# Plachtaa/FAcodec

Hardware: AMD Instinct MI355X
Metric: 24kHz audio sec encoded+decoded per wall-sec (higher is better)
Workload: dtype f32; 1 GPU; configs[1]: batch=32/GPU x 2 s @ 24 kHz, forward encoder->FVQ(6 codebooks)->decoder, FAcodec configs/config.yml model (137.7 M params), weights formula-generated, weight-norm re-materialised every step; clips_per_gpu=32, samples_per_clip=48000, parallelism=dp1 (independent clips, no collective)

## Files before the change

### facodec_amd/_lib.py

```python
import ctypes as C
import os

_HERE = os.path.dirname(os.path.abspath(__file__))
LIB_PATH = os.environ.get("FAC_LIB_PATH", os.path.join(_HERE, "libfacodec_hip.so"))

PAD_ZERO, PAD_REFLECT = 0, 1
ACT_NONE, ACT_TANH, ACT_MISH, ACT_LOG_MEL = 0, 1, 2, 3
ACT_GATE, ACT_WN_RES_SKIP = 4, 5

_p = C.c_void_p
_i = C.c_int
_i64 = C.c_int64
_f = C.c_float


class ConvDesc(C.Structure):
    _fields_ = [
        ("x", _p), ("w", _p), ("bias", _p), ("alpha_in", _p), ("alpha_out", _p), ("res", _p), ("y", _p), ("y2", _p), ("alpha_y2", _p), ("w_k1", _p), ("bias_k1", _p),
        ("x_bs", _i64), ("x_cs", _i64), ("y_bs", _i64), ("y_cs", _i64),
        ("B", C.c_int32), ("C_in", C.c_int32), ("T_in", C.c_int32), ("C_out", C.c_int32),
        ("C_out_pad", C.c_int32), ("T_out", C.c_int32),
        ("K", C.c_int32), ("stride", C.c_int32), ("dilation", C.c_int32), ("pad_left", C.c_int32),
        ("pad_mode", C.c_int32), ("n_phase", C.c_int32), ("y_tstride", C.c_int32), ("phase_shift", C.c_int32),
        ("act", C.c_int32),
        ("w_batched", C.c_int32), ("w_bs", _i64), ("ws", _p), ("ws_bytes", _i64), ("w_split", _p),
        ("K1", C.c_int32), ("dilation2", C.c_int32), ("row_phases", C.c_int32),
        ("x_p8", _p), ("x_p8_plane_bytes", _i64), ("y2_p8", _p), ("y2_p8_plane_bytes", _i64),
        ("pw_split", C.c_int32), ("split_rows", C.c_int32),
        ("gate_cond", _p), ("gate_cond_bs", _i64),
    ]


class VqDesc(C.Structure):
    _fields_ = [
        ("residual", _p), ("z_in", _p), ("zq_acc", _p), ("zq_out", _p), ("w_in", _p), ("b_in", _p),
        ("codebook", _p), ("w_out", _p), ("w_out_scale", _p), ("b_out", _p), ("mask", _p), ("codes", _p), ("z_e", _p),
        ("loss_part", _p), ("codes_bs", _i64),
        ("B", C.c_int32), ("D", C.c_int32), ("T", C.c_int32), ("Kc", C.c_int32),
    ]



VQ_DECODE_MAX_Q = 16


class VqDecodeDesc(C.Structure):
    _fields_ = [
        ("codes", _p * 3), ("codes_bs", _i64 * 3), ("codes_qs", _i64 * 3), ("n_q", C.c_int32 * 3),
        ("codebook", _p * VQ_DECODE_MAX_Q), ("w_out", _p * VQ_DECODE_MAX_Q), ("w_out_scale", _p * VQ_DECODE_MAX_Q),
        ("b_out", _p * VQ_DECODE_MAX_Q), ("style", _p), ("outs", _p), ("z", _p * 3),
        ("B", C.c_int32), ("D", C.c_int32), ("T", C.c_int32), ("Kc", C.c_int32),
# ... 258 lines not shown
```

### facodec_amd/build.py

```python
import os
import subprocess
import sys
from concurrent.futures import ThreadPoolExecutor

HERE = os.path.dirname(os.path.abspath(__file__))
CSRC = os.path.join(HERE, "csrc")
TAG = os.environ.get("FAC_BUILD_TAG", "")
LIB = os.path.join(HERE, "libfacodec_hip%s.so" % ("_" + TAG if TAG else ""))
OBJDIR = "build" + ("_" + TAG if TAG else "")
SOURCES = ["conv1d_api.hip", "conv1d_tile_128x128.hip", "conv1d_tile_96x128.hip", "conv1d_tile_64x128.hip",
           "conv1d_tile_32x256.hip", "conv1d_tile_128x32.hip", "conv1d_tile_128x256.hip", "conv1d_fused_ru.hip", "conv1d_narrow.hip", "conv1d_pw.hip", "conv1d_pw_split.hip", "conv1d_skinny.hip", "conv1d_bsplit.hip", "conv1d_bsplit96.hip", "conv1d_gemm_split.hip", "conv1d_bsplit2.hip", "conv1d_bwd.hip", "conv1d_wgrad_split.hip", "conv1d_wgrad_k1.hip", "train_misc.hip", "optim.hip", "train_quant.hip", "train_pred.hip", "train_disc.hip", "train_redecoder.hip", "pack.hip", "prep_batch.hip", "lstm.hip", "lstm_persist.hip", "vq.hip", "vq_decode.hip", "bitpack.hip", "misc.hip", "attention_stream.hip", "ragged.hip", "resample.hip", "loudness.hip", "metrics.hip", "stream_pool.hip", "jdc.hip", "rccl_arena.hip"]
FLAGS = ["--offload-arch=gfx950", "-O3", "-std=c++17", "-fPIC", "-ffp-contract=off",
         "-Wno-unused-result"] + os.environ.get("FAC_EXTRA_FLAGS", "").split()


def _hipcc():
    for cand in (os.environ.get("HIPCC"), "/opt/rocm/bin/hipcc", "hipcc"):
        if cand and (os.path.isabs(cand) and os.path.exists(cand) or not os.path.isabs(cand)):
            return cand
    return "hipcc"


def _stale(target, deps):
    if not os.path.exists(target):
        return True
    tt = os.path.getmtime(target)
    return any(os.path.getmtime(d) > tt for d in deps)


def build_lib(force=False, verbose=True):
    hipcc = _hipcc()
    headers = sorted(os.path.join(CSRC, f) for f in os.listdir(CSRC) if f.endswith(".h")) + [os.path.join(HERE, "..", "include", "facodec_hip.h")]
    objs, jobs = [], []
    os.makedirs(os.path.join(CSRC, OBJDIR), exist_ok=True)
# ... 23 lines not shown
```

### facodec_amd/convplan.py

```python
from collections import namedtuple

__all__ = ["ConvPlan", "ConvTrPlan", "plan_conv", "plan_convtr", "plan_gemm", "tile_rows", "gemm_split_ok", "gemm_split_strided_ok", "split2_ok",
           "pw_taps_ok", "pw_split_tail_ok", "convtr_split_ok", "convtr_rows_ok", "flat_strided_ok", "flat_convtr_ok", "W_FP32", "W_TAPS",
           "W_GEMM", "W_GEMM_STRIDED", "W_SPLIT2", "W_FP32_PW_TAPS", "PER_CLIP", "FLAT_STRIDED", "FLAT_STRIDE1", "TR_POLYPHASE", "TR_ROWS",
           "TR_ROWS_SPLIT", "TR_ROWS_PW_TAPS", "TR_FLAT"]

W_FP32, W_TAPS, W_GEMM, W_GEMM_STRIDED, W_SPLIT2, W_FP32_PW_TAPS = "fp32", "split_taps", "split_gemm", "split_gemm_strided", "split2", "fp32_pw_taps"
PER_CLIP, FLAT_STRIDED, FLAT_STRIDE1 = "per_clip", "flat_strided", "flat_stride1"
ConvPlan = namedtuple("ConvPlan", "layout form p8")
TR_POLYPHASE, TR_ROWS, TR_ROWS_SPLIT, TR_ROWS_PW_TAPS, TR_FLAT = "polyphase", "rows", "rows_split", "rows_pw_taps", "flat_rows_split"
ConvTrPlan = namedtuple("ConvTrPlan", "layout p8")


def _sw():
    from . import ops
    return ops


def gemm_split_ok(c_out, c_in, k, n_cols, t_out=None):
    sw = _sw()
    if not (sw.BF16_SPLIT and k in (1, 2)):
        return False
    if c_in < sw.GEMM_SPLIT_MIN_CIN or c_out < 64 or n_cols < 1024:
        return False
    return k == 1 or (t_out is not None and t_out >= 256)
# ... 27 lines not shown

def convtr_rows_ok(t_in, stride, causal=True):
    sw = _sw()
    return sw.CONVTR_ROWS and causal and 2 <= stride <= 16 and t_in >= sw.CONVTR_ROWS_MIN_T


def convtr_split_ok(c_in, c_out, stride, batch, t_in, causal=True, alpha_in=None):
    return (_sw().BF16_SPLIT and causal and alpha_in is None and 2 <= stride <= 16 and c_in >= 64
            and t_in >= 256 and batch * t_in >= 1024 and c_out * stride >= 64)


def flat_strided_ok(c_out, c_in, k, s, batch, n_out):
    return (_sw().FLAT_TRAIN and k == 2 * s and s > 1 and n_out < 256 and not gemm_split_strided_ok(c_out, c_in, k, s, batch, n_out)
            and gemm_split_strided_ok(c_out, c_in, k, s, 1, batch * (n_out + 1) - 1))


def flat_convtr_ok(c_in, c_out, s, batch, t_cols):
    return (_sw().FLAT_TRAIN and t_cols < 256 and not convtr_split_ok(c_in, c_out, s, batch, t_cols)
            and convtr_split_ok(c_in, c_out, s, 1, batch * t_cols))


def tile_rows(c_out, c_in, k, grad=False):
    sw = _sw()
    return 96 if (sw.BF16_SPLIT and not grad and k == 7 and c_out in sw.BS_ROWS96 and c_in % 8 == 0) else 64


def plan_conv(c_out, c_in, k, stride, dilation, batch, t_in, t_out, *, k1=0, alpha_in=False, plain=True, res=False,
              causal_reflect=False, grad=True, c_out_mult16=True, split_k=(1, 3, 5, 7), floor_k=(3, 5), tail="pw_split",
              pw_taps=True, split2=False, flat_infer=False, flat_stride1=False, flat_train=None):
    sw = _sw()
    cols = batch * t_out
    p8 = 2.0 * c_out * k / (4.0 * stride)
    if split2 and split2_ok(c_out, k, k1, stride, cols):
        return ConvPlan(W_SPLIT2, PER_CLIP, None)
    if stride > 1:
        strided = not alpha_in and dilation == 1 and not k1
        flat_t = (flat_train is not None and strided and plain and t_in % stride == 0
                  and (flat_train == "zero" or (causal_reflect and t_in > stride))
                  and flat_strided_ok(c_out, c_in, k, stride, batch, t_out))
        if flat_t and flat_train == "reflect":
            return ConvPlan(W_GEMM_STRIDED, FLAT_STRIDED, p8)
        if pw_taps and stride == 2 and strided and plain and pw_taps_ok(c_in, c_out, k, 2, False, batch, t_out):
            return ConvPlan(W_FP32_PW_TAPS, PER_CLIP, None)
        if strided and gemm_split_strided_ok(c_out, c_in, k, stride, batch, t_out):
            return ConvPlan(W_GEMM_STRIDED, PER_CLIP, p8)
        if flat_t:
            return ConvPlan(W_GEMM_STRIDED, FLAT_STRIDED, p8)
# ... 35 lines not shown
```

### facodec_amd/csrc/conv1d_api.hip

```cpp
#include "conv1d_mfma.h"
#include <stdlib.h>

namespace fac {

enum ConvKernel : int {
  CK_128x32 = 0,
  CK_32x256 = 1,
  CK_64x128 = 2,
  CK_96x128 = 3,
  CK_128x128 = 4,
  CK_128x256 = 5,
  CK_96x256 = 6,
  CK_FUSED_RU = 7,
  CK_128x160 = 8,
  CK_NARROW = 9,
  CK_SKINNY = 10,
  CK_BSPLIT = 11,
  CK_CIN1 = 12,
  CK_THIN = 13,
  CK_PW = 14,
  CK_GSPLIT = 15,
  CK_BSPLIT2 = 16,
  CK_PWS = 17,
  CK_PWT = 18,
// ... 41 lines not shown
  FAC_REQUIRE(!d->y2_p8 || d->alpha_y2, "conv1d: y2_p8 needs alpha_y2");
  if (d->w_k1) {
    FAC_REQUIRE(d->C_in == d->C_out && d->C_out_pad == d->C_out && d->n_phase == 1 && d->stride == 1 &&
                    d->alpha_out && d->act == FAC_ACT_NONE && !d->w_batched,
                "conv1d: fused ResidualUnit needs C_in == C_out (multiple of 32), stride 1, a Snake alpha_out");
  }
  a.x_bs = d->x_bs; a.x_cs = d->x_cs; a.y_bs = d->y_bs; a.y_cs = d->y_cs; a.w_bs = d->w_bs;
  a.B = d->B; a.C_in = d->C_in; a.T_in = d->T_in; a.C_out = d->C_out; a.C_out_pad = d->C_out_pad;
  a.T_out = d->T_out; a.K = d->K; a.stride = d->stride; a.dil = d->dilation;
  a.pad_left = d->pad_left; a.pad_mode = d->pad_mode; a.n_phase = d->n_phase;
  a.y_tstride = d->y_tstride; a.act = d->act; a.w_batched = d->w_batched;
  a.phase_shift = d->phase_shift;
  a.rp = d->row_phases > 1 ? d->row_phases : 1;
  FAC_REQUIRE(!d->gate_cond || (d->act == FAC_ACT_GATE && d->gate_cond_bs >= 0),
              "conv1d: gate_cond is the conditioning row of the FAC_ACT_GATE epilogue (act=%d gate_cond_bs=%lld)", d->act,
              (long long)d->gate_cond_bs);
  a.gate_cond = d->gate_cond; a.gate_cond_bs = d->gate_cond_bs;
  if (a.rp > 1) {
    FAC_REQUIRE(d->n_phase == 1 && d->y_tstride == 1 && d->phase_shift == 0 && d->stride == 1 && a.rp <= 128 && !d->w_k1 &&
                    !d->w_batched && d->C_out_pad == fac_convtr_rows(d->C_out, a.rp) && !(d->K1 > 0 && d->K1 < d->K),
                "conv1d: row_phases needs a plain stride-1 launch on weights from fac_pack_convtr_w_rows");
  }
  a.K1 = d->K1 > 0 ? d->K1 : d->K; a.dil2 = d->dilation2;
  FAC_REQUIRE(a.K1 <= d->K && d->K % a.K1 == 0 && (a.K1 == d->K || d->dilation2 > 0), "conv1d: bad two-level taps (K=%d K1=%d)", d->K, d->K1);
  FAC_REQUIRE(!conv_two_level(a) || (!d->w_k1 && d->n_phase == 1 && d->pad_mode == FAC_PAD_ZERO && !d->w_batched),
              "conv1d: two-level taps need a plain, zero-padded conv");
  conv_set_virtual(a);
  FAC_REQUIRE(d->phase_shift >= 0 && d->phase_shift < d->n_phase + (d->n_phase == 1), "conv1d: bad phase_shift");
  {
    long long last = (long long)(d->T_out - 1) * d->stride + (long long)conv_max_tap_offset(a) - d->pad_left;
    int pad_right = last >= d->T_in ? (int)(last - d->T_in + 1) : 0;
    int max_pad = d->pad_left > pad_right ? d->pad_left : pad_right;
    a.T_ext = d->T_in > max_pad ? d->T_in : max_pad + 1;
  }
  if (d->x_p8 || d->y2_p8) {
    const bool gs = d->w_split && (d->K <= 2 || (d->stride > 1 && d->K <= 2 * d->stride)) && conv_gsplit_ok(a) &&
                    !conv_skinny_ok(a, d->ws, d->ws_bytes) && d->C_in % 8 == 0 && d->x_p8_plane_bytes < (1ll << 32);
    const bool ok = !d->y2_p8 && (gs || (d->w_split && !conv_two_level(a) && (d->split_rows == 96 ? conv_bsplit96_p8_ok(a) : conv_bsplit_p8_ok(a)) &&
                                       !conv_cin1_ok(a)));
    FAC_REQUIRE(ok, "conv1d: P8 operands given but the launch does not run on a kernel that takes them (K=%d stride=%d C_in=%d columns=%lld)",
                d->K, d->stride, d->C_in, (long long)d->B * d->T_out);
  }
  if (d->act == FAC_ACT_GATE || d->act == FAC_ACT_WN_RES_SKIP) {
    FAC_REQUIRE(d->w && !d->w_k1 && !d->x_p8 && !conv_two_level(a) && conv_skinny_ok(a, d->ws, d->ws_bytes),
                "conv1d: FAC_ACT_GATE / FAC_ACT_WN_RES_SKIP exist only for few-column launches (B * T_out <= 640) with a workspace");
    k = CK_SKINNY;
// ... 3 lines not shown
  a.gflat = 0;
  a.grt = 0;
  if (d->w_split && (a.KV == 9 || a.KV == 3) && d->C_out <= 32 && conv_bsplit2_ok(a)) {
    a.w = reinterpret_cast<const float*>(d->w_split);
    k = CK_BSPLIT2;
    return FAC_OK;
  }
  FAC_REQUIRE(!conv_two_level(a) || d->w, "conv1d: two-level taps outside the split kernel's shapes need fp32 weights");
  const bool pw_on = pw_enabled();
  if (pw_on && d->pw_split && d->w && conv_pwt_ok(a)) { k = CK_PWT; return FAC_OK; }
  if (d->w_split && (d->K <= 2 || (d->stride > 1 && d->K <= 2 * d->stride)) && conv_gsplit_ok(a) &&
      !conv_skinny_ok(a, d->ws, d->ws_bytes)) {
    a.w = reinterpret_cast<const float*>(d->w_split);
    k = CK_GSPLIT;
    return FAC_OK;
  }
  if (a.rp > 1) {
    FAC_REQUIRE(d->w != nullptr && d->w != (const float*)d->w_split, "conv1d: row_phases launch outside the split kernel's shapes needs fp32 weights");
    k = CK_128x256;
    return FAC_OK;
  }
  const bool two_level = conv_two_level(a);
  FAC_REQUIRE(d->split_rows == 0 || d->split_rows == 64 || d->split_rows == 96, "conv1d: split_rows must be 0, 64 or 96");
  if (d->split_rows == 96) {
    FAC_REQUIRE(d->w_split && !two_level && conv_bsplit96_ok(a) && !conv_cin1_ok(a),
                "conv1d: split_rows = 96 needs a stride-1 k = 7 launch with C_out %% 96 == 0, C_in %% 8 == 0 and more than 640 columns "
                "(K=%d stride=%d C_in=%d C_out=%d columns=%lld)", d->K, d->stride, d->C_in, d->C_out, (long long)d->B * d->T_out);
    a.w = reinterpret_cast<const float*>(d->w_split);
    k = CK_BSPLIT96;
    return FAC_OK;
  }
  if (d->w_split && !two_level && conv_bsplit_ok(a) && !conv_cin1_ok(a)) {
    a.w = reinterpret_cast<const float*>(d->w_split);
    k = CK_BSPLIT;
    return FAC_OK;
  }
  FAC_REQUIRE(d->w != nullptr && (const void*)d->w != d->w_split,
              "conv1d: shape does not qualify for a split-bf16 kernel (K=%d stride=%d C_in=%d C_out=%d columns=%lld) and no fp32 "
              "weights were given", d->K, d->stride, d->C_in, d->C_out, (long long)d->B * d->T_out);
  if (!two_level && conv_skinny_ok(a, d->ws, d->ws_bytes)) k = CK_SKINNY;
  else if (narrow_ok(d) && (!two_level || (a.KV - 1) * a.dil <= 64)) k = CK_NARROW;
  else if (conv_thin_ok(a, d->ws, d->ws_bytes)) k = CK_THIN;
  else if (conv_cin1_ok(a)) k = CK_CIN1;
  else if (pw_on && d->pw_split && conv_pw_ok(a) && conv_pws_ok(a)) k = CK_PWS;
  else if (pw_on && conv_pw_ok(a)) k = CK_PW;
  else k = select_variant(d);
  return FAC_OK;
}

}

// ... 3 lines not shown
  ConvKernel k;
  if (const int rc = conv_plan(d, a, k)) return rc;
  hipStream_t s = (hipStream_t)stream;
  switch (k) {
    case CK_128x32: return conv_dispatch_128x32(a, s);
    case CK_32x256: return conv_dispatch_32x256(a, s);
    case CK_64x128: return conv_dispatch_64x128(a, s);
    case CK_96x128: return conv_dispatch_96x128(a, s);
    case CK_128x128: return conv_dispatch_128x128(a, s);
    case CK_128x256: return conv_dispatch_128x256(a, s);
    case CK_96x256: return conv_dispatch_96x256(a, s);
    case CK_FUSED_RU: return conv_dispatch_fused_ru(a, s);
    case CK_128x160: return conv_dispatch_128x160(a, s);
    case CK_NARROW: return conv_dispatch_narrow(a, s);
    case CK_SKINNY: return conv_dispatch_skinny(a, d->ws, d->ws_bytes, s);
    case CK_BSPLIT: return conv_dispatch_bsplit(a, s);
    case CK_CIN1: return conv_dispatch_cin1(a, s);
    case CK_THIN: return conv_dispatch_thin(a, d->ws, s);
    case CK_PW: return conv_dispatch_pw(a, s);
    case CK_GSPLIT: return conv_dispatch_gsplit(a, s);
    case CK_BSPLIT2: return conv_dispatch_bsplit2(a, s);
    case CK_PWS: return conv_dispatch_pws(a, s);
    case CK_PWT: return conv_dispatch_pwt(a, s);
    case CK_BSPLIT96: return conv_dispatch_bsplit96(a, s);
  }
  return FAC_ERR_ARG;
}

extern "C" int fac_conv1d_variant(const fac_conv_desc* d, char* name, int name_len) {
  using namespace fac;
  ConvArgs a;
  ConvKernel k;
  if (const int rc = conv_plan(d, a, k)) return rc;
  if (!name || name_len <= 0) return k;
  switch (k) {
    case CK_128x32: snprintf(name, name_len, "conv1d_mfma_kernel<1,1,4,1,K> 128x32"); break;
    case CK_32x256: snprintf(name, name_len, "conv1d_mfma_kernel<1,2,1,4,K> 32x256"); break;
    case CK_64x128: snprintf(name, name_len, "conv1d_mfma_kernel<2,1,1,4,K> 64x128"); break;
    case CK_96x128: snprintf(name, name_len, "conv1d_mfma_kernel<3,1,1,4,K> 96x128"); break;
    case CK_128x128: snprintf(name, name_len, "conv1d_mfma_kernel<2,2,2,2,K> 128x128"); break;
    case CK_128x256:
      snprintf(name, name_len, a.rp > 1 ? "conv1d_mfma_kernel<2,2,2,4,2> 128x256 (convtr, all phases per tile)" : "conv1d_mfma_kernel<2,2,2,4,K> 128x256");
      break;
    case CK_96x256: snprintf(name, name_len, "conv1d_mfma_kernel<3,1,1,8,K> 96x256"); break;
    case CK_FUSED_RU: snprintf(name, name_len, "conv1d_mfma_kernel<C/32,1,1,4,7,fused RU> Cx128"); break;
    case CK_128x160: snprintf(name, name_len, "conv1d_mfma_kernel<1,5,4,1,K> 128x160"); break;
    case CK_NARROW:
      snprintf(name, name_len, conv_two_level(a) ? "conv1d_narrow_kernel (VALU, C_out<=2, two-level taps)" : "conv1d_narrow_kernel (VALU, C_out<=2)");
      break;
    case CK_SKINNY:
      snprintf(name, name_len, conv_skinny_single_launch(a) ? "conv1d_gemv_kernel (single launch, <=4 columns)"
                                                            : "conv1d_skinny_kernel (split reduction, <=640 columns)");
      break;
    case CK_BSPLIT: snprintf(name, name_len, "conv1d_bsplit_kernel<%d> 64x256 (bf16x3 split, fp32-grade)", a.K); break;
    case CK_CIN1: snprintf(name, name_len, "conv1d_cin1_kernel (VALU, C_in=1, store stream)"); break;
    case CK_THIN: snprintf(name, name_len, "conv1d_thin_kernel (VALU, C_out<=8, split channels)"); break;
    case CK_PW: snprintf(name, name_len, "conv1d_pw_kernel (k=1 streaming, W in LDS)"); break;
    case CK_GSPLIT:
      snprintf(name, name_len, "conv1d_gemm_split_kernel<%d> 128x128 (bf16x3 split GEMM, fp32-grade)", a.stride > 1 ? 2 : a.K);
      break;
    case CK_BSPLIT2: snprintf(name, name_len, "conv1d_bsplit2_kernel<%d,%d> 32x512 (bf16x3 split, fp32-grade)", a.KV, a.stride); break;
    case CK_PWS: snprintf(name, name_len, "conv1d_pws_kernel (k=1 streaming, W planes in LDS, bf16x3 split, fp32-grade)"); break;
    case CK_PWT: snprintf(name, name_len, "conv1d_pwt_kernel<%d taps> (streaming, W planes in LDS, bf16x3 split, fp32-grade)", a.K); break;
    case CK_BSPLIT96: snprintf(name, name_len, "conv1d_bsplit_kernel<%d> 96x256 (bf16x3 split, fp32-grade)", a.K); break;
  }
  return k;
}
```

### facodec_amd/csrc/conv1d_bsplit_kernel.h

```cpp
#pragma once
#include "conv1d_mfma.h"
#include <type_traits>
#include "inflight_regs.h"
#include "prep_batch.h"

namespace fac {

constexpr int BS_CO = 64;
constexpr int BS96_CO = 96;
constexpr int BS_NSW = 4;
constexpr int BS_NSW_WIDE = 4;
constexpr int BS_XU = 3;
constexpr int BS_WIDE_MIN = 64;
__host__ __device__ constexpr int bs_group(int C_in) { return C_in >= BS_WIDE_MIN ? 2 : 1; }

__host__ __device__ constexpr int bs_slots(int K, int G) { return (G * K + 1) & ~1; }

struct EpiRow {
  float bs, al, inv, a2, i2;
};
__device__ __forceinline__ EpiRow epi_row_load(bool valid, int co, const float* bias, const float* alpha, const float* alpha2) {
  EpiRow r = {0.f, 0.f, 0.f, 0.f, 0.f};
  if (valid) {
    if (bias) r.bs = bias[co];
    if (alpha) { r.al = alpha[co]; r.inv = snake_inv(r.al); }
    if (alpha2) { r.a2 = alpha2[co]; r.i2 = snake_inv(r.a2); }
  }
  return r;
}
__device__ __forceinline__ float epi_row_get(float mine, int lane, int j) {
  return __int_as_float(__builtin_amdgcn_ds_bpermute(((lane & 48) + j) << 2, __float_as_int(mine)));
}

template <int KT, int G, int NMW, int NSW, int MB = 2>
__global__ __launch_bounds__((NMW + NSW) * 64, (NMW + NSW) / 4) void conv1d_bsplit_kernel(ConvArgs a) {
  constexpr int NB = 2;
  constexpr int CO = 32 * MB;
  constexpr bool WIDE = NMW == 4;
  constexpr int BS_TT = 64 * NMW;
  constexpr int H = bs_slots(KT, G);
  constexpr int W_STAGE = 3 * H * CO * 16;
  extern __shared__ __attribute__((aligned(16))) unsigned char sm[];
  const int tid = threadIdx.x;
  const int lane = tid & 63;
  const int wave = __builtin_amdgcn_readfirstlane(tid >> 6);
  const int XW = a.XW;
  const int X_STAGE = 48 * G * XW;
  const int STG = W_STAGE + X_STAGE;
  unsigned char* Wbuf = sm;
  unsigned char* Xbuf = sm + W_STAGE;
  const int n_chunks = (a.C_in + 8 * G - 1) / (8 * G);
  const int dil = a.dil;

  const int n_tiles = a.n_tiles;
  typedef const __attribute__((address_space(4))) ConvArgs* KArgP;
  const KArgP kargs = (KArgP)__builtin_amdgcn_kernarg_segment_ptr();
  auto fresh_args = [&]() {
    KArgP q = kargs;
// ... 7 lines not shown
    const int rest = id / nt;
    const int nb = ka->B;
    b_ = rest % nb;
    co0_ = (rest / nb) * CO;
    t0_ = tt * BS_TT;
  };
  const bool overlap = a.persist != 0;
  unsigned char* epi_base = sm + (overlap ? STG : 0);
  auto walk = [&](auto role) {
  constexpr int ROLE = decltype(role)::value;
  constexpr bool STAGING = ROLE != 0;
  bool first = true;
  unsigned cboff[BS_XU] = {}, nboff[BS_XU] = {};
  unsigned long long cmask[BS_XU] = {}, nmask[BS_XU] = {};
  const float *cxg = nullptr, *nxg = nullptr;
  const unsigned char *cws = nullptr, *nws = nullptr;
  for (int vb = blockIdx.x; vb < n_tiles; vb += gridDim.x) {
  int t0, co0, b;
  decode(fresh_args(), vb, t0, co0, b);
  const bool has_nt = overlap && vb + (int)gridDim.x < n_tiles;

  if constexpr (STAGING) {
    const int lw = wave - NMW;
    __builtin_amdgcn_s_setprio(FAC_PRIO_STAGE);
    const float* xg = a.x + (long long)b * a.x_bs;
    const int xcs = (int)a.x_cs;
    const unsigned char* wsrc = reinterpret_cast<const unsigned char*>(a.w) + (long long)(co0 / CO) * n_chunks * W_STAGE;
    const int n_blk = (XW + 63) >> 6;
    int u_g[BS_XU], u_c[BS_XU], u_idx[BS_XU];
#pragma unroll
    for (int j = 0; j < BS_XU; ++j) {
      const int u = lw + NSW * j;
      u_g[j] = u % G;
      const int c = (u / G) * 64 + lane;
      u_c[j] = (u < G * n_blk && c < XW) ? c : -1;
      const int tin = t0 - a.pad_left + c;
      int idx;
      if (a.pad_mode == FAC_PAD_REFLECT) idx = reflect_index(tin, a.T_in, a.T_ext);
      else idx = (tin >= 0 && tin < a.T_in) ? tin : -1;
      u_idx[j] = u_c[j] >= 0 ? idx : -1;
    }
    constexpr int NBLK = W_STAGE / 1024;
    constexpr int ND = (NBLK + NSW - 1) / NSW;
    constexpr int NX = BS_XU * 8;
    static_assert(W_STAGE % 1024 == 0 && ND + NX <= 63 && NX == 24, "vmcnt is a 6-bit counter; FAC_XREGS24_* list 24 registers per set");
    auto stage_w = [&](int chunk, int buf) {
      constexpr int N16 = W_STAGE / 16;
// ... 188 lines not shown
      float xa[BS_XU][8], xb[BS_XU][8];
      load_x(0, xa);
      stage_w(0, 0);
      if (n_chunks > 1) load_x(1, xb);
      write_x(0, xa);
      __syncthreads();
      for (int chunk = 0; chunk < n_chunks; chunk += 2) {
        if (chunk + 1 < n_chunks) {
          stage_w(chunk + 1, 1);
          if (chunk + 2 < n_chunks) load_x(chunk + 2, xa);
          write_x(1, xb);
        }
        __syncthreads();
        if (chunk + 1 >= n_chunks) break;
        if (chunk + 2 < n_chunks) {
          stage_w(chunk + 2, 0);
          if (chunk + 3 < n_chunks) load_x(chunk + 3, xb);
          write_x(0, xa);
        }
        __syncthreads();
      }
    }
    __builtin_amdgcn_s_setprio(0);
  } else {
  __builtin_amdgcn_s_setprio(FAC_PRIO_MFMA);
  const int l31 = lane & 31;
  const int kq = lane >> 5;
  const int n0 = wave * 64;
  f32x16 acc[MB][NB];
#pragma unroll
  for (int m = 0; m < MB; ++m)
#pragma unroll
    for (int n = 0; n < NB; ++n)
#pragma unroll
      for (int r = 0; r < 16; ++r) acc[m][n][r] = 0.f;

  const int x_lane = (G == 2 ? kq * XW : kq * dil) * 16;
  const int x_step = (G == 2 ? dil : 2 * dil) * 16;

  if (first) __syncthreads();
  if constexpr (NMW == 4) {
    constexpr int S = H / 2;
    auto pipeline = [&](auto MBc) {
    constexpr int MBv = decltype(MBc)::value;
    bf16x8 A[2][MBv][3], Bf[2][NB][3];
    auto ld = [&](int buf, int st, bf16x8 (&Ad)[MBv][3], bf16x8 (&Bd)[NB][3]) {
// ... 99 lines not shown
  }
  __builtin_amdgcn_s_setprio(0);
  {
    float* tile = reinterpret_cast<float*>(epi_base);
    constexpr int EP = BS_TT + 4;
    if constexpr (MB == 3) {
      int lane_off = 4 * kq * EP + n0 + l31;
      asm volatile("" : "+v"(lane_off));
      tile += lane_off;
#pragma unroll
      for (int m = 0; m < MB; ++m)
#pragma unroll
        for (int n = 0; n < NB; ++n)
#pragma unroll
          for (int r = 0; r < 16; ++r) tile[(m * 32 + (r & 3) + 8 * (r >> 2)) * EP + n * 32] = acc[m][n][r];
    } else
#pragma unroll
    for (int m = 0; m < MB; ++m)
#pragma unroll
      for (int n = 0; n < NB; ++n)
#pragma unroll
        for (int r = 0; r < 16; ++r)
          tile[(m * 32 + (r & 3) + 8 * (r >> 2) + 4 * kq) * EP + n0 + n * 32 + l31] = acc[m][n][r];
  }
  }
  __syncthreads();

  {
    const KArgP e = fresh_args();
    const float* tile = reinterpret_cast<const float*>(epi_base);
    constexpr int EP = BS_TT + 4;
    constexpr int NTH = (NMW + NSW) * 64;
    constexpr int QPR = BS_TT / 4;
    float* yg = e->y ? e->y + (long long)b * e->y_bs : nullptr;
    float* y2g = e->y2 ? e->y2 + (long long)b * e->y_bs : nullptr;
    const float* rg = e->res ? e->res + (long long)b * e->y_bs : nullptr;
    const bool vec_ok = (e->y_cs & 3) == 0 && (e->y_bs & 3) == 0 && (!yg || (reinterpret_cast<unsigned long long>(e->y) & 15) == 0) &&
                        (!y2g || (reinterpret_cast<unsigned long long>(e->y2) & 15) == 0) &&
                        (!rg || (reinterpret_cast<unsigned long long>(e->res) & 15) == 0);
    static_assert(QPR % 16 == 0 && NTH % 16 == 0 && (CO * QPR) % 64 == 0 && (CO * QPR + NTH - 1) / NTH <= 16, "EpiRow: 16 lanes share a row, <= 16 iterations");
    const int row_l = (tid + NTH * (lane & 15)) / QPR;
    const EpiRow mine = epi_row_load(row_l < CO && co0 + row_l < e->C_out, co0 + row_l, e->bias, e->alpha_out, y2g ? e->alpha2 : nullptr);
    int j = 0;
    for (int q = tid; q < CO * QPR; q += NTH, ++j) {
      const float bs = epi_row_get(mine.bs, lane, j), al = epi_row_get(mine.al, lane, j), inv = epi_row_get(mine.inv, lane, j);
      float a2 = 0.f, i2 = 0.f;
// ... 36 lines not shown
          if (t + i >= e->T_out) continue;
          if (yg) yg[o + i] = v[i >> 1][i & 1];
          if (y2g) y2g[o + i] = w[i >> 1][i & 1];
        }
      }
    }
  }
  first = !overlap;
  if (vb + (int)gridDim.x < n_tiles) __syncthreads();
  }
  };
  if (wave >= NMW) {
    if constexpr (WIDE) {
      if (a.x_p8 != nullptr) walk(std::integral_constant<int, 2>{});
      else walk(std::integral_constant<int, 1>{});
    } else {
      walk(std::integral_constant<int, 1>{});
    }
  } else {
    walk(std::integral_constant<int, 0>{});
  }
}

template <int KT, int G, int NMW, int NSW, int MB = 2>
static int bsplit_launch(ConvArgs& a, hipStream_t s) {
  constexpr int H = bs_slots(KT, G), TT = 64 * NMW, CO = 32 * MB;
  a.XW = TT + (H / G - 1) * a.dil;
  const size_t stg = (size_t)3 * H * CO * 16 + (size_t)48 * G * a.XW;
  const size_t epi = (size_t)CO * (TT + 4) * sizeof(float);
  a.n_t_tiles = (a.T_out + TT - 1) / TT;
  const long long n_wg = (long long)a.n_t_tiles * ((a.C_out + CO - 1) / CO) * a.B;
  if (n_wg > 0x7fffffffll) {
    set_error("conv1d: too many workgroups (%lld)", n_wg);
    return FAC_ERR_ARG;
  }
  const int n_chunks = (a.C_in + 8 * G - 1) / (8 * G);
  int cus = device_cus() & ~7;
  a.persist = (NMW == 4 && a.x_p8 == nullptr && n_chunks % 2 == 0 && cus >= 8 && n_wg > cus &&
               stg + (stg > epi ? stg : epi) <= FAC_LDS_MAX) ? 1 : 0;
  size_t lds = a.persist ? stg + (stg > epi ? stg : epi) : (2 * stg > epi ? 2 * stg : epi);
  if (lds > FAC_LDS_MAX) {
    set_error("conv1d(bf16 split): tile needs %zu B of LDS (dil=%d)", lds, a.dil);
    return FAC_ERR_ARG;
  }
  constexpr auto kern = conv1d_bsplit_kernel<KT, G, NMW, NSW, MB>;
  allow_dynamic_lds<kern>();
  a.n_tiles = (int)n_wg;
  hipLaunchKernelGGL(kern, dim3((unsigned)(a.persist ? cus : n_wg)), dim3((NMW + NSW) * 64), lds, s, a);
  return check_launch("conv1d_bsplit");
}

}
```

### facodec_amd/csrc/conv1d_mfma.h

```cpp
#pragma once
#include "common.h"

namespace fac {

typedef __attribute__((address_space(3))) void lds_void_t;
typedef __attribute__((address_space(1))) const void glb_void_t;

constexpr int CONV_XMAX = 6;

struct ConvArgs {
  const float* x;
  const float* w;
  const float* bias;
  const float* alpha_in;
  const float* alpha_out;
  const float* res;
  float* y;
  float* y2;
  const float* alpha2;
  const float* w1;
  const float* bias1;
  long long x_bs, x_cs, y_bs, y_cs, w_bs;
  int B, C_in, T_in, T_ext, C_out, C_out_pad, T_out;
  int K, stride, dil, pad_left, pad_mode;
  int n_phase, y_tstride, act, w_batched;
  int phase_shift;
  int K1, dil2;
  int K2v, KV, CV;
  int cic;
  int XW;
  int XB;
  int XQ, XR;
  int n_t_tiles;
  int n_tiles, persist;
  int x_off;
  int gflat;
  int grt;
  const unsigned char* x_p8;
  long long x_p8_ps;
  unsigned char* y2_p8;
  long long y2_p8_ps;
  int rp;
  const float* gate_cond;
  long long gate_cond_bs;
};

__host__ __device__ inline int conv_max_tap_offset(const ConvArgs& a) {
  const int K1 = (a.K1 > 0 && a.K1 < a.K) ? a.K1 : a.K;
  return (a.K / K1 - 1) * a.dil2 + (K1 - 1) * a.dil;
}
__host__ __device__ inline bool conv_two_level(const ConvArgs& a) { return a.K1 > 0 && a.K1 < a.K; }
inline void conv_set_virtual(ConvArgs& a) {
  a.KV = conv_two_level(a) ? a.K1 : a.K;
  a.K2v = a.K / a.KV;
  a.CV = a.C_in * a.K2v;
}

template <int KT>
struct ConvUnroll {
  static constexpr int UC = (KT == 1) ? 4 : ((KT == 2 || KT == 3) ? 2 : 1);
  static constexpr int CIC = KT == 1 ? 24 : (KT == 2 || KT == 3) ? 16 : (KT >= 4 && KT <= 7) ? 8 : (KT > 7 ? 4 : 0);
};

template <int KT, int T_TILE>
constexpr int conv_cic() {
// ... 534 lines not shown
int conv_dispatch_32x256(ConvArgs& a, hipStream_t s);
int conv_dispatch_128x32(ConvArgs& a, hipStream_t s);
int conv_dispatch_128x256(ConvArgs& a, hipStream_t s);
int conv_dispatch_96x256(ConvArgs& a, hipStream_t s);
int conv_dispatch_fused_ru(ConvArgs& a, hipStream_t s);
int conv_dispatch_128x160(ConvArgs& a, hipStream_t s);
int conv_dispatch_narrow(ConvArgs& a, hipStream_t s);
bool conv_cin1_ok(const ConvArgs& a);
bool conv_pw_ok(const ConvArgs& a);
int conv_dispatch_pw(ConvArgs& a, hipStream_t s);
bool conv_thin_ok(const ConvArgs& a, const void* ws, long long ws_bytes);
int conv_dispatch_thin(ConvArgs& a, void* ws, hipStream_t s);
int conv_dispatch_cin1(ConvArgs& a, hipStream_t s);
bool conv_bsplit2_ok(const ConvArgs& a);
int conv_dispatch_bsplit2(ConvArgs& a, hipStream_t s);
bool conv_gsplit_ok(const ConvArgs& a);
int conv_dispatch_gsplit(ConvArgs& a, hipStream_t s);
bool conv_bsplit_ok(const ConvArgs& a);
bool conv_bsplit_p8_ok(const ConvArgs& a);
int conv_dispatch_bsplit(ConvArgs& a, hipStream_t s);
bool conv_bsplit96_ok(const ConvArgs& a);
bool conv_bsplit96_p8_ok(const ConvArgs& a);
int conv_dispatch_bsplit96(ConvArgs& a, hipStream_t s);
bool conv_pws_ok(const ConvArgs& a);
int conv_dispatch_pws(ConvArgs& a, hipStream_t s);
bool conv_pwt_ok(const ConvArgs& a);
int conv_dispatch_pwt(ConvArgs& a, hipStream_t s);
bool conv_skinny_ok(const ConvArgs& a, const void* ws, long long ws_bytes);
bool conv_skinny_single_launch(const ConvArgs& a);
int conv_dispatch_skinny(ConvArgs& a, void* ws, long long ws_bytes, hipStream_t s);

}
```

### facodec_amd/ops.py

```python
import ctypes as C
import math
import os
from collections import namedtuple

import torch

from . import _lib
from .wprep import prepared
from .convplan import *
from ._lib import ConvDesc, VqDesc, VqDecodeDesc, ResampleDesc, PAD_REFLECT, PAD_ZERO, ACT_NONE, ACT_TANH, ACT_MISH, ACT_LOG_MEL, ACT_GATE, ACT_WN_RES_SKIP


def pad32(n):
    return (n + 31) & ~31


def cin_pad(c):
    return ((c + 47) // 48) * 48


_RAW_STREAM = getattr(torch._C, "_cuda_getCurrentRawStream", None)
_GET_DEVICE = getattr(torch._C, "_cuda_getDevice", None)


# ... 151 lines not shown
        global _FLOP_KEY
        self.prev, _FLOP_KEY = _FLOP_KEY, self.key

    def __exit__(self, *a):
        global _FLOP_KEY
        _FLOP_KEY = self.prev


class flop_scale:

    def __init__(self, s):
        self.s = s

    def __enter__(self):
        global _FLOP_SCALE
        self.prev, _FLOP_SCALE = _FLOP_SCALE, self.s

    def __exit__(self, *a):
        global _FLOP_SCALE
        _FLOP_SCALE = self.prev

BF16_SPLIT = True
BS_ROWS96 = (96,)


def set_conv_profile(p):
    global _PROFILE
    _PROFILE = p


_CONV_WS = {}
CONV_WS_BYTES = 32 << 20


_STREAM_SLOTS = {}


def register_stream_slot(stream):
    key = stream.cuda_stream
    if key not in _STREAM_SLOTS:
        _STREAM_SLOTS[key] = len(_STREAM_SLOTS) + 1
    return _STREAM_SLOTS[key]


_SIDE_STREAMS = {}

# ... 212 lines not shown
def to_p8(x, alpha=None):
    x = _dev(x, "x")
    B, C, T = x.shape
    out = P8.empty(B, C, T, x.device)
    _lib.check(_lib.load().fac_to_p8(_ptr(x), _ptr(alpha), _ptr(out.planes), B, C, T, _stream()), "fac_to_p8")
    return out


P8_PREPASS_MIN_FLOP_PER_BYTE = 450.0


def p8_prepass(x, flop_per_in_byte):
    if (flop_per_in_byte is None or P8_PREPASS_MIN_FLOP_PER_BYTE <= 0 or flop_per_in_byte < P8_PREPASS_MIN_FLOP_PER_BYTE or not BF16_SPLIT or isinstance(x, P8)
            or torch.is_grad_enabled() or not x.is_cuda or x.shape[1] % 8 != 0 or x.shape[0] * (x.shape[1] // 8) * x.shape[2] * 16 >= (1 << 32)):
        return x
    return to_p8(x)


def conv_y_channels(c_out, act):
    return c_out // 2 if act in (ACT_GATE, ACT_WN_RES_SKIP) else c_out


def conv_desc(B, c_in, t_in, c_out, k, stride=1, dilation=1, pad_left=None, pad_mode=PAD_REFLECT, t_out=None, act=ACT_NONE, causal=True,
              k1=0, dilation2=0, c_out_pad=None, split_rows=0):
    if pad_left is None:
        t_o, padding_total, _ = conv_out_len(t_in, k, stride, dilation)
        pad_left = padding_total if causal else padding_total - padding_total // 2
        if t_out is None:
            t_out = t_o
    if t_out is None:
        raise ValueError("t_out required with explicit pad_left")
    d = ConvDesc()
    d.x_bs, d.x_cs = c_in * t_in, t_in
    d.y_bs, d.y_cs = conv_y_channels(c_out, act) * t_out, t_out
    d.B, d.C_in, d.T_in, d.C_out, d.C_out_pad, d.T_out = B, c_in, t_in, c_out, (pad32(c_out) if c_out_pad is None else c_out_pad), t_out
    d.K, d.stride, d.dilation, d.pad_left, d.pad_mode = k, stride, dilation, pad_left, pad_mode
    d.n_phase, d.y_tstride, d.act, d.w_batched, d.w_bs = 1, 1, act, 0, 0
    d.K1, d.dilation2, d.split_rows = k1, dilation2, split_rows
    d.pw_split = 1 if (BF16_SPLIT and PW_SPLIT and (k == 1 or (PW_TAPS and k == 4 and stride == 2))) else 0
    return d


def conv1d(x, w_packed, c_out, k, bias=None, stride=1, dilation=1, pad_left=None, pad_mode=PAD_REFLECT,
           t_out=None, alpha_in=None, alpha_out=None, res=None, act=ACT_NONE, out=None, causal=True,
           alpha_y2=None, want_y=True, w_k1=None, bias_k1=None, w_split=None, k1=0, dilation2=0, skip_acc=None, gate_cond=None):
    x_p8 = x if isinstance(x, P8) else None
    if x_p8 is not None:
        B, c_in, t_in = x_p8.shape
    else:
        if not (x.is_cuda and x.dtype == torch.float32 and x.dim() == 3 and x.stride(2) == 1):
            x = _dev(x, "x")
        B, c_in, t_in = x.shape
    dev_ = x_p8.planes.device if x_p8 is not None else x.device
    d = conv_desc(B, c_in, t_in, c_out, k, stride, dilation, pad_left, pad_mode, t_out, act, causal, k1, dilation2,
                  w_packed.shape[-1] if w_packed is not None else None,
                  getattr(w_split, "split_rows", 0))
    t_out, c_y = d.T_out, conv_y_channels(c_out, act)
    if out is None and want_y:
        out = torch.empty(B, c_y, t_out, device=dev_, dtype=torch.float32)
    y2 = torch.empty(B, c_out, t_out, device=dev_, dtype=torch.float32) if alpha_y2 is not None else None
    if act == ACT_WN_RES_SKIP:
# ... 1553 lines not shown
```

### include/facodec_hip.h

```cpp
#ifndef FACODEC_HIP_H
#define FACODEC_HIP_H

#include <stdint.h>

#ifdef __cplusplus
extern "C" {
#endif

typedef void* fac_stream_t;

#define FAC_OK 0
#define FAC_ERR_ARG (-1)
#define FAC_ERR_LAUNCH (-2)

#define FAC_PAD_ZERO 0
#define FAC_PAD_REFLECT 1

#define FAC_ACT_NONE 0
#define FAC_ACT_TANH 1
#define FAC_ACT_MISH 2
#define FAC_ACT_LOG_MEL 3
#define FAC_ACT_GATE 4
#define FAC_ACT_WN_RES_SKIP 5

// ... 33 lines not shown
  const float* bias_k1;
  int64_t x_bs, x_cs;
  int64_t y_bs, y_cs;
  int32_t B, C_in, T_in, C_out, C_out_pad;
  int32_t T_out;
  int32_t K, stride, dilation, pad_left, pad_mode;
  int32_t n_phase;
  int32_t y_tstride;
  int32_t phase_shift;
  int32_t act;
  int32_t w_batched;
  int64_t w_bs;
  void* ws;
  int64_t ws_bytes;
  const void* w_split;
  int32_t K1, dilation2;
  int32_t row_phases;
  const void* x_p8;
  int64_t x_p8_plane_bytes;
  void* y2_p8;
  int64_t y2_p8_plane_bytes;
  int32_t pw_split;
  int32_t split_rows;
  const float* gate_cond;
  int64_t gate_cond_bs;
} fac_conv_desc;

int fac_conv1d_fwd(const fac_conv_desc* d, fac_stream_t stream);
int fac_to_p8(const float* x, const float* alpha, void* out, int B, int C, int T, fac_stream_t stream);
int64_t fac_conv_w_split_bytes(int C_out, int C_in, int K);
int64_t fac_conv_w_split_rows_bytes(int C_out, int C_in, int K, int rows);
int fac_pack_conv_w_split_rows(const float* v, const float* scale, void* out, int C_out, int C_in, int K, int rows, fac_stream_t stream);
int fac_pack_conv_w_split(const float* v, const float* scale, void* out, int C_out, int C_in, int K,
                          fac_stream_t stream);
int64_t fac_conv_w_split2_bytes(int C_out, int C_in, int K, int K1);
int fac_pack_conv_w_split2(const float* v, const float* scale, void* out, int C_out, int C_in, int K, int K1, fac_stream_t stream);
int64_t fac_gemm_w_split_bytes(int R, int C_in, int K, int in_stride);
int fac_pack_gemm_w_split(const float* v, int64_t row_stride, int64_t ci_stride, int64_t k_stride, const float* row_scale, void* out,
                          int R, int C_in, int K, int in_stride, fac_stream_t stream);
int fac_conv1d_variant(const fac_conv_desc* d, char* name, int name_len);

int fac_snake_fwd(const float* x, const float* alpha, float* y, int B, int C, int T,
                  fac_stream_t stream);


int fac_lstm_to_time_major(const float* x, float* xT, int B, int H, int T, fac_stream_t stream);
// ... 357 lines not shown
```

Measured before the change: 1252 audio-s/s.

## Add 16x16x32 bf16 MFMA variant of 96-row bf16x3 split conv kernel

Adds a K32 template variant of the 96x256 bf16x3 split k=7 conv kernel. It uses v_mfma_f32_16x16x32_bf16 with hand-scheduled register double buffering of the A and B fragments, interleaved with LDS loads, in place of the 32x32 MFMA path. Staging and MFMA wave priorities are also changed. Layers with C_out=96 are routed to it by default, which aims to improve MFMA throughput and latency hiding, at the risk of register pressure and more complex scheduling.

```diff
diff --git a/facodec_amd/_lib.py b/facodec_amd/_lib.py
--- a/facodec_amd/_lib.py
+++ b/facodec_amd/_lib.py
@@ -26,7 +26,7 @@
         ("w_batched", C.c_int32), ("w_bs", _i64), ("ws", _p), ("ws_bytes", _i64), ("w_split", _p),
         ("K1", C.c_int32), ("dilation2", C.c_int32), ("row_phases", C.c_int32),
         ("x_p8", _p), ("x_p8_plane_bytes", _i64), ("y2_p8", _p), ("y2_p8_plane_bytes", _i64),
-        ("pw_split", C.c_int32), ("split_rows", C.c_int32),
+        ("pw_split", C.c_int32), ("split_rows", C.c_int32), ("split_k32", C.c_int32),
         ("gate_cond", _p), ("gate_cond_bs", _i64),
     ]
 
diff --git a/facodec_amd/build.py b/facodec_amd/build.py
--- a/facodec_amd/build.py
+++ b/facodec_amd/build.py
@@ -9,7 +9,7 @@
 LIB = os.path.join(HERE, "libfacodec_hip%s.so" % ("_" + TAG if TAG else ""))
 OBJDIR = "build" + ("_" + TAG if TAG else "")
 SOURCES = ["conv1d_api.hip", "conv1d_tile_128x128.hip", "conv1d_tile_96x128.hip", "conv1d_tile_64x128.hip",
-           "conv1d_tile_32x256.hip", "conv1d_tile_128x32.hip", "conv1d_tile_128x256.hip", "conv1d_fused_ru.hip", "conv1d_narrow.hip", "conv1d_pw.hip", "conv1d_pw_split.hip", "conv1d_skinny.hip", "conv1d_bsplit.hip", "conv1d_bsplit96.hip", "conv1d_gemm_split.hip", "conv1d_bsplit2.hip", "conv1d_bwd.hip", "conv1d_wgrad_split.hip", "conv1d_wgrad_k1.hip", "train_misc.hip", "optim.hip", "train_quant.hip", "train_pred.hip", "train_disc.hip", "train_redecoder.hip", "pack.hip", "prep_batch.hip", "lstm.hip", "lstm_persist.hip", "vq.hip", "vq_decode.hip", "bitpack.hip", "misc.hip", "attention_stream.hip", "ragged.hip", "resample.hip", "loudness.hip", "metrics.hip", "stream_pool.hip", "jdc.hip", "rccl_arena.hip"]
+           "conv1d_tile_32x256.hip", "conv1d_tile_128x32.hip", "conv1d_tile_128x256.hip", "conv1d_fused_ru.hip", "conv1d_narrow.hip", "conv1d_pw.hip", "conv1d_pw_split.hip", "conv1d_skinny.hip", "conv1d_bsplit.hip", "conv1d_bsplit96.hip", "conv1d_bsplit96k32.hip", "conv1d_gemm_split.hip", "conv1d_bsplit2.hip", "conv1d_bwd.hip", "conv1d_wgrad_split.hip", "conv1d_wgrad_k1.hip", "train_misc.hip", "optim.hip", "train_quant.hip", "train_pred.hip", "train_disc.hip", "train_redecoder.hip", "pack.hip", "prep_batch.hip", "lstm.hip", "lstm_persist.hip", "vq.hip", "vq_decode.hip", "bitpack.hip", "misc.hip", "attention_stream.hip", "ragged.hip", "resample.hip", "loudness.hip", "metrics.hip", "stream_pool.hip", "jdc.hip", "rccl_arena.hip"]
 FLAGS = ["--offload-arch=gfx950", "-O3", "-std=c++17", "-fPIC", "-ffp-contract=off",
          "-Wno-unused-result"] + os.environ.get("FAC_EXTRA_FLAGS", "").split()
 
diff --git a/facodec_amd/convplan.py b/facodec_amd/convplan.py
--- a/facodec_amd/convplan.py
+++ b/facodec_amd/convplan.py
@@ -1,6 +1,6 @@
 from collections import namedtuple
 
-__all__ = ["ConvPlan", "ConvTrPlan", "plan_conv", "plan_convtr", "plan_gemm", "tile_rows", "gemm_split_ok", "gemm_split_strided_ok", "split2_ok",
+__all__ = ["ConvPlan", "ConvTrPlan", "plan_conv", "plan_convtr", "plan_gemm", "tile_rows", "rows96_k32", "gemm_split_ok", "gemm_split_strided_ok", "split2_ok",
            "pw_taps_ok", "pw_split_tail_ok", "convtr_split_ok", "convtr_rows_ok", "flat_strided_ok", "flat_convtr_ok", "W_FP32", "W_TAPS",
            "W_GEMM", "W_GEMM_STRIDED", "W_SPLIT2", "W_FP32_PW_TAPS", "PER_CLIP", "FLAT_STRIDED", "FLAT_STRIDE1", "TR_POLYPHASE", "TR_ROWS",
            "TR_ROWS_SPLIT", "TR_ROWS_PW_TAPS", "TR_FLAT"]
@@ -74,7 +74,11 @@
 
 def tile_rows(c_out, c_in, k, grad=False):
     sw = _sw()
-    return 96 if (sw.BF16_SPLIT and not grad and k == 7 and c_out in sw.BS_ROWS96 and c_in % 8 == 0) else 64
+    return 96 if (sw.BF16_SPLIT and not grad and k == 7 and (c_out in sw.BS_ROWS96 or c_out in sw.BS_ROWS96_WIDE) and c_in % 8 == 0) else 64
+
+
+def rows96_k32(c_out):
+    return c_out in _sw().BS_ROWS96_K32
 
 
 def plan_conv(c_out, c_in, k, stride, dilation, batch, t_in, t_out, *, k1=0, alpha_in=False, plain=True, res=False,
diff --git a/facodec_amd/csrc/conv1d_api.hip b/facodec_amd/csrc/conv1d_api.hip
--- a/facodec_amd/csrc/conv1d_api.hip
+++ b/facodec_amd/csrc/conv1d_api.hip
@@ -87,6 +87,7 @@
                 "conv1d: row_phases needs a plain stride-1 launch on weights from fac_pack_convtr_w_rows");
   }
   a.K1 = d->K1 > 0 ? d->K1 : d->K; a.dil2 = d->dilation2;
+  a.k32 = 0;
   FAC_REQUIRE(a.K1 <= d->K && d->K % a.K1 == 0 && (a.K1 == d->K || d->dilation2 > 0), "conv1d: bad two-level taps (K=%d K1=%d)", d->K, d->K1);
   FAC_REQUIRE(!conv_two_level(a) || (!d->w_k1 && d->n_phase == 1 && d->pad_mode == FAC_PAD_ZERO && !d->w_batched),
               "conv1d: two-level taps need a plain, zero-padded conv");
@@ -136,11 +137,13 @@
   }
   const bool two_level = conv_two_level(a);
   FAC_REQUIRE(d->split_rows == 0 || d->split_rows == 64 || d->split_rows == 96, "conv1d: split_rows must be 0, 64 or 96");
+  FAC_REQUIRE(d->split_k32 == 0 || (d->split_k32 == 1 && d->split_rows == 96), "conv1d: split_k32 is 0 or 1 and belongs to split_rows = 96");
   if (d->split_rows == 96) {
     FAC_REQUIRE(d->w_split && !two_level && conv_bsplit96_ok(a) && !conv_cin1_ok(a),
                 "conv1d: split_rows = 96 needs a stride-1 k = 7 launch with C_out %% 96 == 0, C_in %% 8 == 0 and more than 640 columns "
                 "(K=%d stride=%d C_in=%d C_out=%d columns=%lld)", d->K, d->stride, d->C_in, d->C_out, (long long)d->B * d->T_out);
     a.w = reinterpret_cast<const float*>(d->w_split);
+    a.k32 = d->split_k32;
     k = CK_BSPLIT96;
     return FAC_OK;
   }
@@ -190,7 +193,7 @@
     case CK_BSPLIT2: return conv_dispatch_bsplit2(a, s);
     case CK_PWS: return conv_dispatch_pws(a, s);
     case CK_PWT: return conv_dispatch_pwt(a, s);
-    case CK_BSPLIT96: return conv_dispatch_bsplit96(a, s);
+    case CK_BSPLIT96: return a.k32 ? conv_dispatch_bsplit96k32(a, s) : conv_dispatch_bsplit96(a, s);
   }
   return FAC_ERR_ARG;
 }
@@ -230,7 +233,9 @@
     case CK_BSPLIT2: snprintf(name, name_len, "conv1d_bsplit2_kernel<%d,%d> 32x512 (bf16x3 split, fp32-grade)", a.KV, a.stride); break;
     case CK_PWS: snprintf(name, name_len, "conv1d_pws_kernel (k=1 streaming, W planes in LDS, bf16x3 split, fp32-grade)"); break;
     case CK_PWT: snprintf(name, name_len, "conv1d_pwt_kernel<%d taps> (streaming, W planes in LDS, bf16x3 split, fp32-grade)", a.K); break;
-    case CK_BSPLIT96: snprintf(name, name_len, "conv1d_bsplit_kernel<%d> 96x256 (bf16x3 split, fp32-grade)", a.K); break;
+    case CK_BSPLIT96:
+      snprintf(name, name_len, a.k32 ? "conv1d_bsplit_kernel<%d> 96x256 (bf16x3 k32 split, fp32-grade)" : "conv1d_bsplit_kernel<%d> 96x256 (bf16x3 split, fp32-grade)", a.K);
+      break;
   }
   return k;
 }
diff --git a/facodec_amd/csrc/conv1d_bsplit96k32.hip b/facodec_amd/csrc/conv1d_bsplit96k32.hip
--- /dev/null
+++ b/facodec_amd/csrc/conv1d_bsplit96k32.hip
@@ -0,0 +1,7 @@
+#include "conv1d_bsplit_kernel.h"
+
+namespace fac {
+
+int conv_dispatch_bsplit96k32(ConvArgs& a, hipStream_t s) { return bsplit_launch<7, 1, 4, BS_NSW_WIDE, 3, true>(a, s); }
+
+}
diff --git a/facodec_amd/csrc/conv1d_bsplit_kernel.h b/facodec_amd/csrc/conv1d_bsplit_kernel.h
--- a/facodec_amd/csrc/conv1d_bsplit_kernel.h
+++ b/facodec_amd/csrc/conv1d_bsplit_kernel.h
@@ -32,8 +32,9 @@
   return __int_as_float(__builtin_amdgcn_ds_bpermute(((lane & 48) + j) << 2, __float_as_int(mine)));
 }
 
-template <int KT, int G, int NMW, int NSW, int MB = 2>
+template <int KT, int G, int NMW, int NSW, int MB = 2, bool K32 = false>
 __global__ __launch_bounds__((NMW + NSW) * 64, (NMW + NSW) / 4) void conv1d_bsplit_kernel(ConvArgs a) {
+  static_assert(!K32 || (KT == 7 && G == 1 && NMW == 4 && MB == 3), "K32: the 96-row form of the k = 7 kernel only");
   constexpr int NB = 2;
   constexpr int CO = 32 * MB;
   constexpr bool WIDE = NMW == 4;
@@ -87,7 +88,7 @@
 
   if constexpr (STAGING) {
     const int lw = wave - NMW;
-    __builtin_amdgcn_s_setprio(FAC_PRIO_STAGE);
+    __builtin_amdgcn_s_setprio(K32 ? 1 : FAC_PRIO_STAGE);
     const float* xg = a.x + (long long)b * a.x_bs;
     const int xcs = (int)a.x_cs;
     const unsigned char* wsrc = reinterpret_cast<const unsigned char*>(a.w) + (long long)(co0 / CO) * n_chunks * W_STAGE;
@@ -322,6 +323,97 @@
       }
     }
     __builtin_amdgcn_s_setprio(0);
+  } else {
+  if constexpr (K32) {
+  static_assert(H == 8, "K32: two steps of four half slots");
+  __builtin_amdgcn_s_setprio(3);
+  const int l15 = lane & 15;
+  const int kg = lane >> 4;
+  const int n0 = wave * 64;
+  f32x4 acc[6][4];
+#pragma unroll
+  for (int m = 0; m < 6; ++m)
+#pragma unroll
+    for (int n = 0; n < 4; ++n) acc[m][n] = f32x4{0.f, 0.f, 0.f, 0.f};
+  const int w_lane = (kg * CO + l15) * 16;
+  const int x_lane = (n0 + l15 + kg * dil) * 16;
+  const int x_step = 4 * dil * 16;
+  if (first) __syncthreads();
+  typedef f32x4 frag;
+  frag SA[3][6], SB[3][4];
+  auto pA = [&](int boff, int st, int plane) {
+    int wl = w_lane;
+    asm volatile("" : "+v"(wl));
+    return reinterpret_cast<const frag*>(Wbuf + boff + wl + (plane * H + 4 * st) * CO * 16);
+  };
+  auto pB = [&](int boff, int st, int plane) {
+    int xl = x_lane;
+    asm volatile("" : "+v"(xl));
+    return reinterpret_cast<const frag*>(Xbuf + boff + xl + st * x_step + plane * XW * 16);
+  };
+#define BS_MFMA16(ACC, AF, BF) asm volatile("v_mfma_f32_16x16x32_bf16 %0, %1, %2, %0" : "+v"(ACC) : "v"(AF), "v"(BF) : "memory")
+  auto phase = [&](const frag (&Ac)[6], const frag (&Bc)[4], auto n1c, frag* dst1, const frag* src1, auto n2c, frag* dst2, const frag* src2) {
+    constexpr int N1 = decltype(n1c)::value, N2 = decltype(n2c)::value, EVERY = N1 + N2 > 6 ? 1 : 2;
+#pragma unroll
+    for (int i = 0; i < 24; ++i) {
+      BS_MFMA16(acc[i >> 2][i & 3], Ac[i >> 2], Bc[i & 3]);
+      const int r = (i + 1) % EVERY == 0 ? (i + 1) / EVERY - 1 : N1 + N2;
+      if (r < N1) dst1[r] = src1[r * 16];
+      else if (r < N1 + N2) dst2[r - N1] = src2[(r - N1) * 16];
+    }
+  };
+  using std::integral_constant;
+  constexpr integral_constant<int, 0> none{};
+  auto step = [&](auto stc, int cur, int nxt) {
+    constexpr int st = decltype(stc)::value, nst = 1 - st;
+    constexpr int b_hi = 1 + st, b_lo = 2 - st;
+    constexpr integral_constant<int, 6> nA{};
+    constexpr integral_constant<int, 4> nB{};
+    phase(SA[1], SB[0], nA, SA[0], pA(cur, st, 0), nB, SB[b_lo], pB(cur, st, 2));
+    if constexpr (st == 1) {
+      asm volatile("s_waitcnt lgkmcnt(0)" ::: "memory");
+      __builtin_amdgcn_s_barrier();
+      asm volatile("" ::: "memory");
+    }
+    phase(SA[2], SB[b_hi], none, nullptr, nullptr, none, nullptr, nullptr);
+    phase(SA[0], SB[b_lo], none, nullptr, nullptr, none, nullptr, nullptr);
+    phase(SA[1], SB[b_hi], nB, SB[b_lo], pB(nxt, nst, 0), none, nullptr, nullptr);
+    phase(SA[0], SB[0], nA, SA[1], pA(nxt, nst, 1), none, nullptr, nullptr);
+    phase(SA[0], SB[b_hi], nB, SB[0], pB(nxt, nst, 1), nA, SA[2], pA(nxt, nst, 2));
+  };
+  {
+    const frag *q0 = pB(0, 0, 1), *q1 = pA(0, 0, 1), *q2 = pB(0, 0, 0), *q3 = pA(0, 0, 2);
+#pragma unroll
+    for (int n = 0; n < 4; ++n) SB[0][n] = q0[n * 16];
+#pragma unroll
+    for (int m = 0; m < 6; ++m) SA[1][m] = q1[m * 16];
+#pragma unroll
+    for (int n = 0; n < 4; ++n) SB[1][n] = q2[n * 16];
+#pragma unroll
+    for (int m = 0; m < 6; ++m) SA[2][m] = q3[m * 16];
+  }
+  asm volatile("s_nop 4" ::: "memory");
+  for (int chunk = 0; chunk < n_chunks; ++chunk) {
+    const int cur = (chunk & 1) * STG, nxt = STG - cur;
+    step(integral_constant<int, 0>{}, cur, cur);
+    step(integral_constant<int, 1>{}, cur, nxt);
+  }
+  asm volatile("s_nop 15\n\ts_nop 15" ::: "memory");
+#undef BS_MFMA16
+  __builtin_amdgcn_s_setprio(0);
+  {
+    float* tile = reinterpret_cast<float*>(epi_base);
+    constexpr int EP = BS_TT + 4;
+    int lane_off = 4 * kg * EP + n0 + l15;
+    asm volatile("" : "+v"(lane_off));
+    tile += lane_off;
+#pragma unroll
+    for (int m = 0; m < 6; ++m)
+#pragma unroll
+      for (int n = 0; n < 4; ++n)
+#pragma unroll
+        for (int i = 0; i < 4; ++i) tile[(m * 16 + i) * EP + n * 16] = acc[m][n][i];
+  }
   } else {
   __builtin_amdgcn_s_setprio(FAC_PRIO_MFMA);
   const int l31 = lane & 31;
@@ -467,6 +559,7 @@
 #pragma unroll
         for (int r = 0; r < 16; ++r)
           tile[(m * 32 + (r & 3) + 8 * (r >> 2) + 4 * kq) * EP + n0 + n * 32 + l31] = acc[m][n][r];
+  }
   }
   }
   __syncthreads();
@@ -549,7 +642,7 @@
   }
 }
 
-template <int KT, int G, int NMW, int NSW, int MB = 2>
+template <int KT, int G, int NMW, int NSW, int MB = 2, bool K32 = false>
 static int bsplit_launch(ConvArgs& a, hipStream_t s) {
   constexpr int H = bs_slots(KT, G), TT = 64 * NMW, CO = 32 * MB;
   a.XW = TT + (H / G - 1) * a.dil;
@@ -570,7 +663,7 @@
     set_error("conv1d(bf16 split): tile needs %zu B of LDS (dil=%d)", lds, a.dil);
     return FAC_ERR_ARG;
   }
-  constexpr auto kern = conv1d_bsplit_kernel<KT, G, NMW, NSW, MB>;
+  constexpr auto kern = conv1d_bsplit_kernel<KT, G, NMW, NSW, MB, K32>;
   allow_dynamic_lds<kern>();
   a.n_tiles = (int)n_wg;
   hipLaunchKernelGGL(kern, dim3((unsigned)(a.persist ? cus : n_wg)), dim3((NMW + NSW) * 64), lds, s, a);
diff --git a/facodec_amd/csrc/conv1d_mfma.h b/facodec_amd/csrc/conv1d_mfma.h
--- a/facodec_amd/csrc/conv1d_mfma.h
+++ b/facodec_amd/csrc/conv1d_mfma.h
@@ -41,6 +41,7 @@
   unsigned char* y2_p8;
   long long y2_p8_ps;
   int rp;
+  int k32;
   const float* gate_cond;
   long long gate_cond_bs;
 };
@@ -621,6 +622,7 @@
 bool conv_bsplit96_ok(const ConvArgs& a);
 bool conv_bsplit96_p8_ok(const ConvArgs& a);
 int conv_dispatch_bsplit96(ConvArgs& a, hipStream_t s);
+int conv_dispatch_bsplit96k32(ConvArgs& a, hipStream_t s);
 bool conv_pws_ok(const ConvArgs& a);
 int conv_dispatch_pws(ConvArgs& a, hipStream_t s);
 bool conv_pwt_ok(const ConvArgs& a);
diff --git a/facodec_amd/ops.py b/facodec_amd/ops.py
--- a/facodec_amd/ops.py
+++ b/facodec_amd/ops.py
@@ -197,6 +197,8 @@
 
 BF16_SPLIT = True
 BS_ROWS96 = (96,)
+BS_ROWS96_WIDE = ()
+BS_ROWS96_K32 = (96,)
 
 
 def set_conv_profile(p):
@@ -455,7 +457,7 @@
 
 
 def conv_desc(B, c_in, t_in, c_out, k, stride=1, dilation=1, pad_left=None, pad_mode=PAD_REFLECT, t_out=None, act=ACT_NONE, causal=True,
-              k1=0, dilation2=0, c_out_pad=None, split_rows=0):
+              k1=0, dilation2=0, c_out_pad=None, split_rows=0, split_k32=None):
     if pad_left is None:
         t_o, padding_total, _ = conv_out_len(t_in, k, stride, dilation)
         pad_left = padding_total if causal else padding_total - padding_total // 2
@@ -469,7 +471,9 @@
     d.B, d.C_in, d.T_in, d.C_out, d.C_out_pad, d.T_out = B, c_in, t_in, c_out, (pad32(c_out) if c_out_pad is None else c_out_pad), t_out
     d.K, d.stride, d.dilation, d.pad_left, d.pad_mode = k, stride, dilation, pad_left, pad_mode
     d.n_phase, d.y_tstride, d.act, d.w_batched, d.w_bs = 1, 1, act, 0, 0
-    d.K1, d.dilation2, d.split_rows = k1, dilation2, split_rows
+    if split_k32 is None:
+        split_k32 = 1 if split_rows == 96 and rows96_k32(c_out) else 0
+    d.K1, d.dilation2, d.split_rows, d.split_k32 = k1, dilation2, split_rows, split_k32
     d.pw_split = 1 if (BF16_SPLIT and PW_SPLIT and (k == 1 or (PW_TAPS and k == 4 and stride == 2))) else 0
     return d
 
diff --git a/include/facodec_hip.h b/include/facodec_hip.h
--- a/include/facodec_hip.h
+++ b/include/facodec_hip.h
@@ -79,6 +79,7 @@
   int64_t y2_p8_plane_bytes;
   int32_t pw_split;
   int32_t split_rows;
+  int32_t split_k32;
   const float* gate_cond;
   int64_t gate_cond_bs;
 } fac_conv_desc;
```

New measurement: 1256 audio-s/s (median of 6 runs). No clear change (+0.3%).
